# ronantakizawa/cudabulletproof

Measured on AMD Instinct MI355X. Metric: 64-bit range-proof verifies/sec (batched), higher is better.
Workload: dtype u64

## Files before the change

### cudabulletproof_amd/csrc/bp_capi.hip

```cpp
#include <hip/hip_runtime.h>
#include <map>
#include <tuple>
#include <mutex>
#include <string>
#include <vector>
#include <cstdio>
#include <cstdlib>
#include <cstring>
#include <algorithm>
#include <chrono>
#include <thread>

#include "../../include/cudabulletproof_hip.h"
#include "bp_kernels.h"
#include "ge25519_dev.h"

static_assert(sizeof(fe25519) == 32, "fe25519 layout");
static_assert(sizeof(ge25519) == 128, "ge25519 layout");
static_assert(sizeof(bp::fe) == 32 && sizeof(bp::ge) == 128, "device layout");
static_assert(sizeof(InnerProductProof) == 144, "InnerProductProof layout (SURVEY 8b)");
static_assert(sizeof(RangeProof) == 880, "RangeProof layout (SURVEY 8b)");

namespace {

// ... 290 lines not shown
    bp::SlotDev* host_dev = nullptr;
    int head = 0;

    struct Stages {
        int ft, m3, fin;
    };
    Stages stages(int L) const {
        Stages g;
        g.ft = L > 0 ? L + 1 : 1;
        g.m3 = range_mode == 2 ? (g.ft > 3 ? g.ft : 3) : -1;
        int last = g.ft;
        if (range_mode && last < 2) last = 2;
        if (g.m3 > last) last = g.m3;
        g.fin = last + 1;
        return g;
    }
    bool lane_tree = false, chains_first = false;
    bool defer_msm = false;
    int quad_force = -1;
    unsigned long long row_max = ROW_MAX_ITEMS, quad_max = QUAD_MAX_ITEMS, pair_max = PAIR_MAX_ITEMS;
    static constexpr size_t LANE_SORT_MIN = 64;
    bool lane_sort = true;
    int lane_sort_mask = 7;
    Buf sort_bins, sort_offs;
    bp::LaneSortPlan plan{};
    hipStream_t sort_s = nullptr;
    hipEvent_t ev_tick = nullptr, ev_sorted = nullptr;
    Buf ptab;
    const bp::ge* ext_tab = nullptr;
    int pbits = 0;
    const bp::ge* tables() const { return ext_tab ? ext_tab : ptab.as<bp::ge>(); }
    hipError_t init(Engine* eng, hipStream_t st, size_t mb, int nn, int range) {
        e = eng; s = st; maxB = mb; n = nn; range_mode = range;
        const char* ls = getenv("HIPBP_LANE_SORT");
        lane_sort_mask = ls ? atoi(ls) : 7;
        lane_sort = (lane_sort_mask & 7) != 0;
        const char* lt = getenv("HIPBP_LANE_TREE_MAX");
        lane_tree = n <= (lt ? atoi(lt) : bp::LANE_TREE_MAX);
        const char* cf = getenv("HIPBP_CHAINS_FIRST");
        chains_first = cf ? atoi(cf) != 0 : false;
        const char* qe = getenv("HIPBP_QUAD");
        const char* qm = getenv("HIPBP_QUAD_MAX_ITEMS");
        const char* pm = getenv("HIPBP_PAIR_MAX_ITEMS");
        quad_force = qe ? (atoi(qe) == 1 ? 4 : atoi(qe) == 2 ? 2 : atoi(qe) == 3 ? 16 : 1) : -1;
        const char* rm = getenv("HIPBP_ROW_MAX_ITEMS");
        row_max = rm ? strtoull(rm, nullptr, 10) : ROW_MAX_ITEMS;
        quad_max = qm ? strtoull(qm, nullptr, 10) : QUAD_MAX_ITEMS;
        pair_max = pm ? strtoull(pm, nullptr, 10) : PAIR_MAX_ITEMS;
        const char* dm = getenv("HIPBP_DEFER_MSM");
        defer_msm = dm && atoi(dm) != 0;
        if (const char* sp = getenv("HIPBP_DEFER_SPAN")) {
            int a = 2, b = 1, c = 0;
            if (sscanf(sp, "%d:%d:%d", &a, &b, &c) >= 1 && a >= 2) {
                defer_first = a;
                defer_last_off = b < 0 ? 0 : b;
                defer_weight = c != 0;
            }
        }
        Lr = log2i((size_t)n);
        D = stages(Lr).fin + 1;
        slots.resize(D);
        hipError_t r;
        if ((r = hipMalloc(&slots_dev, D * sizeof(bp::SlotDev))) != hipSuccess) return r;
        if ((r = hipHostMalloc(&host_dev, D * sizeof(bp::SlotDev))) != hipSuccess) return r;
        for (auto& sl : slots)
            if ((r = hipEventCreateWithFlags(&sl.copied, hipEventDisableTiming)) != hipSuccess) return r;
        const char* ss = getenv("HIPBP_SORT_STREAM");
        if (ss && atoi(ss) != 0) {
            int lo_pr = 0, hi_pr = 0;
            if ((r = hipDeviceGetStreamPriorityRange(&lo_pr, &hi_pr)) != hipSuccess) return r;
            if ((r = hipStreamCreateWithPriority(&sort_s, hipStreamNonBlocking, hi_pr)) != hipSuccess) return r;
            if ((r = hipEventCreateWithFlags(&ev_tick, hipEventDisableTiming)) != hipSuccess) return r;
            if ((r = hipEventCreateWithFlags(&ev_sorted, hipEventDisableTiming)) != hipSuccess) return r;
        }
        return hipSuccess;
    }
    void release() {
        if (s) (void)hipStreamSynchronize(s);
        for (auto& sl : slots) {
            for (auto& b : sl.b) if (b.p) (void)hipFree(b.p);
            if (sl.copied) (void)hipEventDestroy(sl.copied);
        }
        if (slots_dev) (void)hipFree(slots_dev);
        if (host_dev) (void)hipHostFree(host_dev);
        if (sort_s) (void)hipStreamSynchronize(sort_s);
        if (sort_s) (void)hipStreamDestroy(sort_s);
        if (ev_tick) (void)hipEventDestroy(ev_tick);
        if (ev_sorted) (void)hipEventDestroy(ev_sorted);
        if (sort_bins.p) (void)hipFree(sort_bins.p);
        if (sort_offs.p) (void)hipFree(sort_offs.p);
        if (ptab.p) (void)hipFree(ptab.p);
    }
    hipError_t plan_sort(Slot& sl, int idx) {
        plan = bp::LaneSortPlan{};
        bp::SlotDev& d = sl.dev;
        d.perm0 = nullptr;
        for (auto& q : d.permr) q = nullptr;
        d.perm_ft = nullptr;
        const unsigned long long B = d.bv.B;
        const int L = d.bv.L_len;
        if (!lane_sort || B < LANE_SORT_MIN) return hipSuccess;
        struct S { int kind, r; unsigned long long items; };
        S sets[bp::LANE_SORT_SETS];
        int cnt = 0;
        const bp::Stage0Lanes z = bp::stage0_lanes(B, n, L, range_mode);
        for (int c = 0; c < 4; c++)
            if (z.size[c] && (lane_sort_mask & 1)) sets[cnt++] = {bp::SS_STAGE0, c, z.size[c]};
        for (int r = 1; r < L; r++)
            if (bp::round_per_lane(n, r) && (lane_sort_mask & 2))
                sets[cnt++] = {bp::SS_ROUND, r, B * 4 * (unsigned long long)(n >> (r + 1))};
        if (lane_sort_mask & 4) sets[cnt++] = {bp::SS_FT, 0, B * 2};
        if (!cnt) return hipSuccess;
        plan.longest_first = (lane_sort_mask & 8) ? 0 : 1;
        unsigned long long total = 0;
        for (int k = 0; k < cnt; k++) total += sets[k].items;
        if (total > 0xFFFFFFFFull) return hipSuccess;
        hipError_t r;
        if ((r = sl.b[20].need(total * sizeof(uint32_t))) != hipSuccess) return r;
        const size_t nb = (size_t)bp::LANE_SORT_SETS * bp::MSM_BINS * sizeof(unsigned);
        if (!sort_bins.p) {
            if ((r = sort_bins.need(nb)) != hipSuccess) return r;
            if ((r = hipMemsetAsync(sort_bins.p, 0, nb, s)) != hipSuccess) return r;
            if ((r = sort_offs.need(nb)) != hipSuccess) return r;
        }
        uint32_t* base = sl.b[20].as<uint32_t>();
        unsigned blk = 0;
        for (int k = 0; k < cnt; k++) {
            bp::LaneSortPlan::Set& st = plan.set[k];
            st.kind = sets[k].kind; st.r = sets[k].r; st.items = sets[k].items; st.perm = base; st.block0 = blk;
            if (st.kind == bp::SS_STAGE0 && !d.perm0) d.perm0 = base;
            else if (st.kind == bp::SS_ROUND) d.permr[st.r] = base;
            else d.perm_ft = base;
            base += sets[k].items;
            blk += (unsigned)((sets[k].items + bp::LANE_SORT_BLOCK - 1) / bp::LANE_SORT_BLOCK);
        }
        plan.count = cnt;
        plan.blocks = blk;
        plan.slot = slots_dev + idx;
        return hipSuccess;
    }
    bool busy() const {
        for (auto& sl : slots) if (sl.active) return true;
        return false;
    }
    bool defer_ok() const { return range_mode != 0 && lane_tree && Lr >= 2 && 2 * Lr + 5 <= bp::MAX_REGIONS; }
    int defer_first = 2, defer_last_off = 0, defer_weight = 0;
    int msm_last(int L) const { return L - defer_last_off > defer_first ? L - defer_last_off : defer_first; }
    void msm_chunk(unsigned long long total, int L, int st, unsigned long long& lo, unsigned long long& hi) const {
        const int m = msm_last(L) - defer_first + 1, k = st - defer_first;
        auto cut = [&](int j) -> unsigned long long {
            if (j >= m) return total;
            const unsigned long long num = defer_weight ? (1ull << j) - 1 : (unsigned long long)j;
            const unsigned long long den = defer_weight ? (1ull << m) - 1 : (unsigned long long)m;
            return (total / 64 * num / den) * 64;
        };
        lo = cut(k);
        hi = cut(k + 1);
    }
    int ltree_stage(const Slot& sl, const Stages& g) const {
        return sl.dev.defer ? msm_last(sl.dev.bv.L_len) + 1 : std::min(3, g.fin - 1);
    }
// ... 28 lines not shown
    int push(const hipbp_proof_batch* b, const ge25519* P_in, uint8_t* ok, ge25519* P_out, ge25519* chk,
             uint8_t* flags_out = nullptr, ge25519* poly_out = nullptr) {
        EventTimer* tm = e->timer.on ? &e->timer : nullptr;
        bool has = b && b->count > 0;
        Slot& nw = slots[head];
        if (has) {
            int rc = check_batch(b, range_mode);
            if (rc != HIPBP_OK) return rc;
            if ((int)b->n != n) { g_err = "batch n differs from the pipeline's"; return HIPBP_ERR_ARG; }
            if (nw.active) { g_err = "pipeline slot busy (internal)"; return HIPBP_ERR_ARG; }
            BP_RET_ON(carve(nw, b->count, b->L_len));
            nw.dev.bv = view_of(b);
            nw.dev.ok = ok;
            nw.dev.P_out = (bp::ge*)P_out;
            nw.dev.chk_out = (bp::ge*)chk;
            nw.dev.flags_out = flags_out;
            nw.dev.poly_out = (bp::ge*)poly_out;
            nw.dev.range_mode = range_mode;
            nw.dev.lane_tree = lane_tree ? 1 : 0;
            nw.dev.ptab = pbits ? tables() : nullptr;
            nw.dev.pbits = pbits;
            nw.dev.defer = (defer_msm && defer_ok() && (int)b->L_len >= 2 &&
                            msm_last((int)b->L_len) + 1 < stages((int)b->L_len).fin) ? 1 : 0;
            BP_RET_ON(plan_sort(nw, head));
            BP_RET_ON(hipEventSynchronize(nw.copied));
            host_dev[head] = nw.dev;
            BP_RET_ON(hipMemcpyAsync(slots_dev + head, host_dev + head, sizeof(bp::SlotDev), hipMemcpyHostToDevice, s));
            BP_RET_ON(hipEventRecord(nw.copied, s));
            if (!range_mode)
                BP_RET_ON(hipMemcpyAsync(nw.dev.ws.Pin, P_in, b->count * sizeof(ge25519), hipMemcpyDeviceToDevice, s));
            nw.active = true;
            nw.stage = 0;
            nw.B = b->count;
        }
        bp::RegionList tr{};
        bool overflow = false;
        auto add = [&overflow](bp::RegionList& rl, int kind, int slot, int r, unsigned long long items, unsigned align) {
            if (!items) return;
            if (rl.count == bp::MAX_REGIONS) { overflow = true; return; }
            bp::Region& g = rl.reg[rl.count++];
            g.kind = kind; g.slot = slot; g.r = r; g.begin = rl.total; g.items = items;
            rl.total += (items + align - 1) & ~(unsigned long long)(align - 1);
        };
        const int chain_pass = chains_first ? 1 : 3;
        for (int pass = 0; pass < 4; pass++) {
            for (int k = 0; k < D; k++) {
                int idx = (head - k + D) % D;
// ... 18 lines not shown
                    }
                    if (st >= 2 && st <= L) add(tr, bp::RK_ROUND, idx, st - 1, B * 4 * (n >> st), 64);
                    if (sl.dev.defer && st >= defer_first && st <= msm_last(L)) {
                        unsigned long long lo, hi;
                        msm_chunk(bp::stage0_lanes(B, n, L, range_mode, bp::S0_DEFER).total, L, st, lo, hi);
                        add(tr, bp::RK_MSMT, idx, (int)lo, hi - lo, 64);
                    }
                    if (st == g.ft) add(tr, bp::RK_FINAL_TERMS, idx, 0, B * 2, 64);
                    if (st == g.m3) add(tr, bp::RK_M3, idx, 0, B * 2, 64);
                }
            }
        }
        if (overflow) { g_err = "pipeline region list overflow (internal)"; return HIPBP_ERR_ARG; }
        unsigned long long sm_items = 0;
        for (int k = 0; k < tr.count; k++)
            if (bp::region_is_sm(tr.reg[k].kind)) sm_items += tr.reg[k].items;
        int ql = sm_items <= row_max ? 16 : sm_items <= quad_max ? 4 : sm_items <= pair_max ? 2 : 1;
        if (!sm_items) {
            unsigned long long chain_items = 0;
            for (int k = 0; k < tr.count; k++) chain_items += tr.reg[k].items;
            ql = chain_items <= row_max ? 16 : 4;
        }
        if (quad_force >= 0) ql = quad_force;
        if (ql > 1) {
            unsigned long long tot = 0;
            for (int k = 0; k < tr.count; k++) {
                bp::Region& g = tr.reg[k];
                g.items *= bp::region_lanes(g.kind, ql);
                g.begin = tot;
                const unsigned long long al = g.kind == bp::RK_TREE ? 256 : 64;
                tot += (g.items + al - 1) & ~(al - 1);
            }
            tr.total = tot;
        }
        if (tr.total >= (1ull << 32)) { g_err = "pipeline tick exceeds 2^32 lanes (batch too large for n)"; return HIPBP_ERR_ARG; }
        if (tm) tm->mark(bp::KT_TERMS, false, s);
        bp::launch_terms(tr, slots_dev, G, H, g ? g : h, h, e->dtab, e->two_i, s, ql);
        if (tm) tm->mark(bp::KT_TERMS, true, s);
        BP_RET_ON(hipGetLastError());
        if (has && plan.count) {
            if (sort_s) {
                BP_RET_ON(hipEventRecord(ev_tick, s));
                BP_RET_ON(hipStreamWaitEvent(sort_s, ev_tick, 0));
                bp::launch_lane_sort(plan, sort_bins.as<unsigned>(), sort_offs.as<unsigned>(), sort_s);
                BP_RET_ON(hipGetLastError());
                BP_RET_ON(hipEventRecord(ev_sorted, sort_s));
                BP_RET_ON(hipStreamWaitEvent(s, ev_sorted, 0));
            } else {
                bp::launch_lane_sort(plan, sort_bins.as<unsigned>(), sort_offs.as<unsigned>(), s);
                BP_RET_ON(hipGetLastError());
            }
        }
        for (auto& sl : slots) {
            if (!sl.active) continue;
            if (sl.stage == stages(sl.dev.bv.L_len).fin) sl.active = false;
            else sl.stage++;
        }
        head = (head + 1) % D;
        return HIPBP_OK;
    }
    int flush() {
        while (busy()) {
            int rc = push(nullptr, nullptr, nullptr, nullptr, nullptr);
            if (rc != HIPBP_OK) return rc;
        }
        return HIPBP_OK;
    }
};

hipError_t msm_run(Engine& e, bp::ge* results, const bp::fe* scalars, const bp::ge* points, size_t n, size_t count,
                   hipStream_t s, const bp::ge* ptab = nullptr, int K = 0) {
    const size_t tot = n * count, nb = count * ((n + 255) / 256);
    Buf* w = e.msm_bufs(s);
    hipError_t err;
    if ((err = w[0].need(tot * sizeof(bp::ge))) != hipSuccess) return err;
// ... 1424 lines not shown
```

### cudabulletproof_amd/csrc/bp_kernels.h

```cpp
#pragma once
#include <hip/hip_runtime.h>
#include <stddef.h>
#include <stdint.h>

namespace bp {
struct fe;
struct ge;

struct BatchView {
    int B;
    int n;
    int ab_len;
    int L_len;
    const ge* V;
    const ge* A;
    const ge* S;
    const ge* T1;
    const ge* T2;
    const fe* t;
    const fe* a;
    const fe* b;
    const fe* c;
    const fe* x;
    const ge* L;
// ... 18 lines not shown
    ge* Pin;
    fe* psc;
    ge* pterm;
    ge* lr;
    fe* chal;
    ge* m3;
    uint8_t* rflags;
    ge* pbase;
};

struct SlotDev {
    BatchView bv;
    VerifyWs ws;
    uint8_t* ok;
    ge* P_out;
    ge* chk_out;
    uint8_t* flags_out;
    ge* poly_out;
    int range_mode;
    int lane_tree;
    uint32_t* perm0;
    uint32_t* permr[17];
    uint32_t* perm_ft;
    const ge* ptab;
    int pbits;
    int defer;
};

struct Stage0Lanes {
    unsigned long long U;
    unsigned long long off[4], size[4];
    unsigned long long total;
    unsigned long long pl;
};
enum Stage0Sel { S0_ALL = 0, S0_CRIT = 1, S0_DEFER = 2 };
__host__ __device__ inline Stage0Lanes stage0_lanes(unsigned long long B, int n, int L, int range_mode, int sel = S0_ALL) {
    Stage0Lanes z;
    const unsigned long long msm = range_mode ? B * 2 * n : 0, fold = L > 0 ? B * 2 * n : 0;
    const bool uni = n >= 64;
    const bool m = sel != S0_CRIT, f = sel != S0_DEFER;
    z.U = uni ? (m ? msm / 2 : 0) + (f ? fold : 0) : 0;
    z.size[0] = m ? (uni ? msm / 2 : msm) : 0;
    z.size[1] = f && !uni ? fold : 0;
    z.size[2] = m ? B * 2 : 0;
    z.size[3] = f && range_mode == 2 ? B * 7 : 0;
    unsigned long long o = z.U, pl = 0;
// ... 23 lines not shown
    const int n = sd.bv.n, ln = log2n(n);
    const Stage0Lanes z = stage0_lanes(B, n, sd.bv.L_len, sd.range_mode, sel);
    if (l < (uint32_t)z.U) {
        const uint32_t nG = (sd.range_mode && sel != S0_CRIT) ? B << ln : 0;
        if (l < nG) return ((l >> ln) << (ln + 1)) + (l & (n - 1));
        return (sd.range_mode ? B << (ln + 1) : 0) + (l - nG);
    }
    const Stage0Lanes za = sel == S0_ALL ? z : stage0_lanes(B, n, sd.bv.L_len, sd.range_mode);
    int c = 0;
    uint32_t base = 0;
#pragma unroll
    for (int k = 1; k < 4; k++)
        if (l >= (uint32_t)z.off[k]) { c = k; base += (uint32_t)za.size[k - 1]; }
    const uint32_t j = l - (uint32_t)z.off[c];
    if (j >= (uint32_t)z.size[c]) return UINT32_MAX;
    return stage0_class_item(sd, c, sd.perm0 ? sd.perm0[base + j] : j);
}

__host__ __device__ inline bool round_per_lane(int n, int r) { return (n >> r) < 64; }

constexpr int MSM_BINS = 513;

enum SortSetKind { SS_STAGE0 = 0, SS_ROUND = 1, SS_FT = 2 };
constexpr int LANE_SORT_SETS = 18;
constexpr int LANE_SORT_BLOCK = 256;
struct LaneSortPlan {
    int count;
    int pad;
    const SlotDev* slot;
    struct Set {
        int kind, r;
        unsigned long long items;
        uint32_t* perm;
        unsigned block0;
        unsigned pad;
    } set[LANE_SORT_SETS];
    unsigned blocks;
    int longest_first;
};
void launch_lane_sort(const LaneSortPlan& plan, unsigned* bins, unsigned* offs, hipStream_t s);

enum RegionKind { RK_STAGE0 = 0, RK_ROUND = 1, RK_FINAL_TERMS = 2, RK_FINAL = 4, RK_PREP = 5,
                  RK_TREE = 6, RK_POLY = 7, RK_M3 = 8,
                  RK_LTREE = 9 ,
                  RK_MSMT = 10  };
struct Region {
    int kind;
    int slot;
    int r;
    int pad;
    unsigned long long begin;
    unsigned long long items;
};
constexpr int LANE_TREE_MAX = 64;
constexpr int MAX_REGIONS = 24;
struct RegionList {
    int count;
    int pad;
    unsigned long long total;
    Region reg[MAX_REGIONS];
};

enum KernelKind { KT_PREP = 0, KT_TERMS, KT_TREE, KT_COMBINE, KT_COUNT };

void launch_prefix_tables(ge* tab, const ge* G, const ge* H, const ge* h, const ge* g, int n, int K, hipStream_t s);
void launch_terms(const RegionList& rl, const SlotDev* slots, const ge* G, const ge* H, const ge* g, const ge* h,
                  const ge* dtab, const fe* two_i, hipStream_t s, int ql = 1);
void launch_upload(void* dst, const void* src, size_t bytes, hipStream_t s);
#define BP_DECL_TERMS(Q)                                                                                    \
    void launch_terms##Q(const RegionList& rl, const SlotDev* slots, const ge* G, const ge* H, const ge* g,  \
                         const ge* h, const ge* dtab, const fe* two_i, hipStream_t s, unsigned lds_pad);
BP_DECL_TERMS(1)
BP_DECL_TERMS(2)
BP_DECL_TERMS(4)
BP_DECL_TERMS(16)
#undef BP_DECL_TERMS
inline bool region_is_sm(int kind) {
    return kind == RK_STAGE0 || kind == RK_ROUND || kind == RK_FINAL_TERMS || kind == RK_M3 || kind == RK_MSMT;
}
inline int region_lanes(int kind, int ql) {
    if (region_is_sm(kind)) return ql;
    return (ql >= 4 && (kind == RK_FINAL || kind == RK_LTREE || kind == RK_PREP)) ? 4 : 1;
}

constexpr size_t MSM_SORT_MIN = 4096;
void launch_msm_points(ge* pts, const fe* scal, const ge* P, size_t m, uint32_t* perm, unsigned* bins,
                       const ge* dtab, hipStream_t s, size_t pm = 0, const ge* ptab = nullptr, int K = 0);
void launch_tree(ge* out, const ge* in, int S, size_t m, hipStream_t s);
void launch_ops_scan(unsigned* bins, int longest_first, hipStream_t s);
hipError_t msm_pippenger(ge* result, const fe* scal, const ge* P, size_t n, size_t count, int c, const ge* dtab,
                         hipStream_t s);
hipError_t msm_pippenger_windows(ge* Sw, const fe* scal, const ge* P, size_t n, int c, int w0, int w1,
                                 const ge* dtab, hipStream_t s);
hipError_t pippenger_horner(ge* result, const ge* Sw, size_t count, int c, hipStream_t s);
hipError_t pippenger_release(hipStream_t s);



struct ProveIn {
    int B, n, L;
    const fe* v;
    const fe* gamma;
    const fe* sL;
    const fe* sR;
    const fe* rnd;
// ... 74 lines not shown
```

### cudabulletproof_amd/csrc/bp_kernels.hip

```cpp
#include "bp_kernels.h"
#include "ge25519_dev.h"
#include "ge25519_quad.h"
#include "sha256_dev.h"

namespace bp {

constexpr int TPB = 256;
#ifndef BP_TERMS_OCC
#define BP_TERMS_OCC 4
#endif


__device__ __forceinline__ size_t gid() { return (size_t)blockIdx.x * blockDim.x + threadIdx.x; }

__global__ __launch_bounds__(TPB) void k_prefix_tables(ge* tab, const ge* __restrict__ G, const ge* __restrict__ H,
                                                       const ge* __restrict__ h, const ge* __restrict__ g, int n,
                                                       int K, size_t total) {
    const size_t i = gid();
    if (i >= total) return;
    const size_t b = i >> K;
    const uint32_t p = (uint32_t)(i & ((1ull << K) - 1));
    const ge* P = b < (size_t)n ? &G[b] : b < 2 * (size_t)n ? &H[b - n] : b == 2 * (size_t)n ? h : g;
    if (!P) return;
    const geq q = ge_prep(*P);
// ... 105 lines not shown
}

__global__ __launch_bounds__(TPB) void k_tree(ge* out, const ge* __restrict__ in, size_t m, int nb) {
    __shared__ ge sh[TPB];
    int seg = blockIdx.x / nb, chunk = blockIdx.x % nb;
    int tid = threadIdx.x;
    size_t base = (size_t)seg * m + (size_t)chunk * TPB;
    int cnt = (int)min((size_t)TPB, m - (size_t)chunk * TPB);
    if (tid < cnt) sh[tid] = in[base + tid];
    __syncthreads();
    for (int st = 1; st < cnt; st <<= 1) {
        const int i = 2 * st * tid;
        if (i + st < cnt) sh[i] = ge_norm_dev(ge_add(sh[i], sh[i + st]));
        __syncthreads();
    }
    if (tid == 0) out[blockIdx.x] = sh[0];
}

void launch_tree(ge* out, const ge* in, int S, size_t m, hipStream_t s) {
    int nb = (int)((m + TPB - 1) / TPB);
    k_tree<<<S * nb, TPB, 0, s>>>(out, in, m, nb);
}

__device__ __forceinline__ int lane_key(const SlotDev& sd, int kind, int r, size_t j) {
    const BatchView& bv = sd.bv;
    const VerifyWs& ws = sd.ws;
    const size_t B = bv.B;
    const int n = bv.n, Lr = bv.L_len;
    fe s;
    int K = 0;
    if (kind == SS_STAGE0) {
        size_t i = stage0_class_item(sd, r, (uint32_t)j);
        if (sd.ptab) K = sd.pbits;
        const size_t nA = sd.range_mode ? B * 2 * n : 0, nB = Lr > 0 ? B * 2 * n : 0;
        if (i < nA) {
            size_t seg = i / n, p = seg >> 1;
            s = (seg & 1) ? ws.sH[p * n + i % n] : ws.sG[p];
        } else if (i - nA < nB) {
            i -= nA;
            size_t p = i / (2 * n);
            int grp = (int)(i % (2 * n)) / (n >> 1);
            s = grp < 2 ? ws.uinv[p * Lr] : ws.u[p * Lr];
        } else if (i - nA - nB < 2 * B) {
            i -= nA + nB;
            bool isC = i & 1;
            if (!isC && !sd.range_mode) return 0;
            s = ws.sc[(i >> 1) * 4 + (isC ? 3 : 0)];
        } else {
            i -= nA + nB + 2 * B;
            s = ws.psc[(i / 7) * 8 + i % 7];
            const int k = (int)(i % 7);
            if (k == 2 || k == 5 || k == 6) K = 0;
        }
    } else if (kind == SS_ROUND) {
        const int np = n >> (r + 1);
        size_t p = j / (4 * np);
        int grp = (int)(j % (4 * np)) / np;
        s = grp < 2 ? ws.uinv[p * Lr + r] : ws.u[p * Lr + r];
    } else {
        s = ws.sc[(j >> 1) * 4 + ((j & 1) ? 2 : 1)];
    }
    return sm_ops_prefix(s, K);
}

__device__ __forceinline__ int lane_set_of(const LaneSortPlan& pl, unsigned b, LaneSortPlan::Set& st) {
    int idx = 0;
    st = pl.set[0];
#pragma unroll
    for (int k = 1; k < LANE_SORT_SETS; k++)
        if (k < pl.count && b >= pl.set[k].block0) { st = pl.set[k]; idx = k; }
    return idx;
}

__global__ __launch_bounds__(LANE_SORT_BLOCK) void k_lane_hist(LaneSortPlan pl, unsigned* bins) {
    __shared__ unsigned h[OPS_BINS];
    for (int k = threadIdx.x; k < OPS_BINS; k += LANE_SORT_BLOCK) h[k] = 0;
    __syncthreads();
    LaneSortPlan::Set st;
    const int si = lane_set_of(pl, blockIdx.x, st);
    const size_t j = (size_t)(blockIdx.x - st.block0) * LANE_SORT_BLOCK + threadIdx.x;
    if (j < st.items) atomicAdd(&h[lane_key(*pl.slot, st.kind, st.r, j)], 1u);
    __syncthreads();
    for (int k = threadIdx.x; k < OPS_BINS; k += LANE_SORT_BLOCK)
        if (h[k]) atomicAdd(&bins[si * OPS_BINS + k], h[k]);
}

constexpr int LS_PER = (OPS_BINS + LANE_SORT_BLOCK - 1) / LANE_SORT_BLOCK;
__global__ __launch_bounds__(LANE_SORT_BLOCK) void k_lane_scan(unsigned* bins, unsigned* offs, int longest_first) {
    __shared__ unsigned wsum[LANE_SORT_BLOCK / 64];
    const int t = threadIdx.x;
    unsigned* bb = bins + (size_t)blockIdx.x * OPS_BINS;
    unsigned v[LS_PER], sum = 0;
#pragma unroll
    for (int u = 0; u < LS_PER; u++) {
        const int p = LS_PER * t + u, k = longest_first ? OPS_BINS - 1 - p : p;
        v[u] = p < OPS_BINS ? bb[k] : 0u;
        sum += v[u];
    }
    unsigned inc = sum;
#pragma unroll
    for (int d = 1; d < 64; d <<= 1) {
        const unsigned x = __shfl_up(inc, d, 64);
        if ((t & 63) >= d) inc += x;
    }
    if ((t & 63) == 63) wsum[t >> 6] = inc;
    __syncthreads();
    unsigned run = inc - sum;
    for (int w = 0; w < (t >> 6); w++) run += wsum[w];
#pragma unroll
    for (int u = 0; u < LS_PER; u++) {
        const int p = LS_PER * t + u, k = longest_first ? OPS_BINS - 1 - p : p;
        if (p < OPS_BINS) {
            offs[(size_t)blockIdx.x * OPS_BINS + k] = run;
            bb[k] = 0;
        }
        run += v[u];
    }
}

__global__ __launch_bounds__(LANE_SORT_BLOCK) void k_lane_scatter(LaneSortPlan pl, unsigned* offs) {
    __shared__ unsigned cnt[OPS_BINS], base[OPS_BINS];
    for (int k = threadIdx.x; k < OPS_BINS; k += LANE_SORT_BLOCK) cnt[k] = 0;
    __syncthreads();
    LaneSortPlan::Set st;
    const int si = lane_set_of(pl, blockIdx.x, st);
    const size_t j = (size_t)(blockIdx.x - st.block0) * LANE_SORT_BLOCK + threadIdx.x;
    int key = 0;
    unsigned rank = 0;
    if (j < st.items) {
        key = lane_key(*pl.slot, st.kind, st.r, j);
        rank = atomicAdd(&cnt[key], 1u);
    }
    __syncthreads();
    for (int k = threadIdx.x; k < OPS_BINS; k += LANE_SORT_BLOCK)
        if (cnt[k]) base[k] = atomicAdd(&offs[si * OPS_BINS + k], cnt[k]);
    __syncthreads();
    if (j < st.items) st.perm[base[key] + rank] = (uint32_t)j;
}

void launch_lane_sort(const LaneSortPlan& plan, unsigned* bins, unsigned* offs, hipStream_t s) {
    if (!plan.count || !plan.blocks) return;
    k_lane_hist<<<plan.blocks, LANE_SORT_BLOCK, 0, s>>>(plan, bins);
    k_lane_scan<<<plan.count, LANE_SORT_BLOCK, 0, s>>>(bins, offs, plan.longest_first);
    k_lane_scatter<<<plan.blocks, LANE_SORT_BLOCK, 0, s>>>(plan, offs);
}

static inline unsigned nblk(size_t items) { return (unsigned)((items + TPB - 1) / TPB); }

void launch_terms(const RegionList& rl, const SlotDev* slots, const ge* G, const ge* H, const ge* g, const ge* h,
                  const ge* dtab, const fe* two_i, hipStream_t s, int ql) {
    if (!rl.total) return;
    static const unsigned pad = [] { const char* e = getenv("HIPBP_TERMS_LDS_PAD"); return e ? (unsigned)atoi(e) : 0u; }();
    if (ql == 16) launch_terms16(rl, slots, G, H, g, h, dtab, two_i, s, pad);
    else if (ql == 4) launch_terms4(rl, slots, G, H, g, h, dtab, two_i, s, pad);
    else if (ql == 2) launch_terms2(rl, slots, G, H, g, h, dtab, two_i, s, pad);
    else launch_terms1(rl, slots, G, H, g, h, dtab, two_i, s, pad);
}


__global__ __launch_bounds__(TPB) void k_field_op(int op, fe* r, const fe* __restrict__ a, const fe* __restrict__ b,
                                                  size_t count) {
    size_t i = gid();
    if (op == 10 || op == 12) {
        i >>= 2;
        if (i >= count) return;
        const fe z = op == 10 ? fe_mul_q4(a[i], b[i]) : fe_mul_q4_k(a[i]);
        if ((threadIdx.x & 3) == 0) r[i] = z;
        return;
    }
// ... 219 lines not shown
```

### cudabulletproof_amd/csrc/bp_verify_dev.h

```cpp
#pragma once
#include "bp_kernels.h"
#include "ge25519_dev.h"
#include "ge25519_quad.h"
#include "sha256_dev.h"

namespace bp {

#ifndef BP_TERMS_OCC
#define BP_TERMS_OCC 4
#endif
constexpr int TPB = 256;
__device__ __forceinline__ size_t gid() { return (size_t)blockIdx.x * blockDim.x + threadIdx.x; }



__device__ __forceinline__ void prep_std_task(const BatchView& bv, const VerifyWs& ws, const fe* __restrict__ two_i,
                                              size_t p, const fe& z, const fe& z2, const fe& sy) {
    const int n = bv.n;
    fe x = chal_x(bv.T1[p], bv.T2[p]);
    const fe two = fe_add(fe_set(1), fe_set(1));
    fe z3 = fe_mul(z2, z);
    fe t1 = fe_mul(fe_sub(z, z2), sy);
    fe s2 = fe_set(1);
    for (int i = 1; i < n; i++) s2 = fe_add(s2, two_i[i]);
// ... 114 lines not shown
            tr = u;
        }
        const bool me = (r & 3) == qd;
        const int k = r >> 2;
        m0 = fe_sel(me && k == 0, u, m0);
        m1 = fe_sel(me && k == 1, u, m1);
        m2 = fe_sel(me && k == 2, u, m2);
        m3 = fe_sel(me && k == 3, u, m3);
    }
#pragma unroll
    for (int k = 0; k < 4; k++) {
        const int r = 4 * k + qd;
        const fe u = k == 0 ? m0 : k == 1 ? m1 : k == 2 ? m2 : m3;
        if (r < Lr) {
            ws.u[p * Lr + r] = fe_canon(u);
            ws.uinv[p * Lr + r] = fe_canon(fe_invert(u));
        }
    }
    if (qd == 0) {
        ws.ipok[p] = fe_eq(fe_canon(acc), fe_canon(bv.c[p])) ? 1 : 0;
        ws.sc[p * 4 + 1] = fe_canon(bv.a[p * abl]);
        ws.sc[p * 4 + 2] = fe_canon(bv.b[p * abl]);
        ws.sc[p * 4 + 3] = fe_canon(bv.c[p]);
    }
}

__device__ __forceinline__ ge folded_point(const VerifyWs& ws, int n, int r, size_t p, bool isH, int m) {
    const int npp = n >> r;
    const ge* f = ws.fold[(r - 1) & 1] + p * (2 * n);
    if (!isH) return ge_norm_host(ge_add(f[m], f[2 * npp + m]));
    return ge_norm_host(ge_add(f[3 * npp + m], f[npp + m]));
}

struct SmJob {
    fe s;
    ge P;
    ge* dst;
    int dev_norm;
    int base;
};


__device__ __forceinline__ void fold_job(const BatchView& bv, const VerifyWs& ws, int r, uint32_t p, uint32_t k,
                                         const ge* __restrict__ G, const ge* __restrict__ H, SmJob& jb) {
    const int n = bv.n, lnp = log2n(n) - r - 1, np = 1 << lnp, Lr = bv.L_len;
    const int grp = (int)(k >> lnp), j = (int)(k & (np - 1));
// ... 250 lines not shown
    if (i >= rl.total) return;
    const Region rg = find_region(rl, i);
    size_t l = i - rg.begin;
    const SlotDev& sd = slots[rg.slot];
    if (rg.kind == RK_TREE) {
        ge* sh = reinterpret_cast<ge*>(qs);
        const int n = sd.bv.n, ch = n < TPB ? n : TPB, tid = threadIdx.x, idx = tid & (ch - 1);
        const bool live = l < rg.items;
        if (live) sh[tid] = sd.ws.msm_pts[l];
        __syncthreads();
        for (int st = 1; st < ch; st <<= 1) {
            const int j = tid - idx + 2 * st * idx;
            if (live && 2 * st * idx + st < ch) sh[j] = ge_norm_dev(ge_add(sh[j], sh[j + st]));
            __syncthreads();
        }
        if (live && idx == 0) {
            if (n <= TPB) sd.ws.msm_part[l / n] = sh[tid];
            else sd.ws.msm_pts[l] = sh[tid];
        }
        return;
    }
    if (l >= rg.items) return;
    if (rg.kind == RK_PREP) {
        const size_t B = sd.bv.B;
        if (QL >= 4) {
            const size_t it = l >> 2;
            const int qd = threadIdx.x & 3;
            if (sd.range_mode && it < B) prep_range_task_q4(sd.bv, sd.ws, two_i, it, sd.range_mode, qd);
            else prep_ipa_task_q4(sd.bv, sd.ws, sd.range_mode ? it - B : it, qd);
        } else if (sd.range_mode && l < B) {
            prep_range_task(sd.bv, sd.ws, two_i, l, sd.range_mode);
        } else {
            prep_ipa_task(sd.bv, sd.ws, sd.range_mode ? l - B : l);
        }
    } else if (rg.kind == RK_POLY) {
        poly_task(sd, l);
    } else if (rg.kind == RK_FINAL) {
        if (QL >= 4) final_task<true>(sd, l >> 2);
        else final_task<false>(sd, l);
    } else if (rg.kind == RK_LTREE) {
        if (QL >= 4) ltree_task<true>(sd, l >> 2);
        else ltree_task<false>(sd, l);
    } else {
        SmJob jb;
        jb.base = -1;
        bool live = true;
        uint32_t li = (uint32_t)l;
        if (QL == 16) li >>= 4;
        if (QL == 4) li >>= 2;
        if (QL == 2) li >>= 1;
        if (rg.kind == RK_STAGE0 || rg.kind == RK_MSMT) {
            const uint32_t it = rg.kind == RK_MSMT ? stage0_item(sd, (uint32_t)rg.r + li, S0_DEFER)
                                                   : stage0_item(sd, li, sd.defer ? S0_CRIT : S0_ALL);
            live = it != UINT32_MAX && stage0_job(sd, it, G, H, g, h, jb);
        } else if (rg.kind == RK_M3) {
            m3_job(sd, li, jb);
// ... 37 lines not shown
```

Before: 210,200.

## Fuse lane-sort permutation building into prep kernel with per-block local sort

Drops the separate histogram, scan and scatter lane-sort kernels and their global bin buffers and optional side stream. Each prep block now sorts the MSM lanes of its own group of proofs in LDS, right after the prep work, and writes the permutation directly. Prep lanes are re-laid out as whole 256-thread groups split into range and IPA parts, so every thread reaches the block barriers. This saves three launches and the global atomics per step. In exchange the ordering becomes block-local rather than batch-wide, and the serial per-set sort loop lengthens the prep kernel.

New measurement: 210,600 (median of 6 runs). No clear change (+0.2%).

```diff
diff --git a/cudabulletproof_amd/csrc/bp_capi.hip b/cudabulletproof_amd/csrc/bp_capi.hip
--- a/cudabulletproof_amd/csrc/bp_capi.hip
+++ b/cudabulletproof_amd/csrc/bp_capi.hip
@@ -336,10 +336,6 @@
     static constexpr size_t LANE_SORT_MIN = 64;
     bool lane_sort = true;
     int lane_sort_mask = 7;
-    Buf sort_bins, sort_offs;
-    bp::LaneSortPlan plan{};
-    hipStream_t sort_s = nullptr;
-    hipEvent_t ev_tick = nullptr, ev_sorted = nullptr;
     Buf ptab;
     const bp::ge* ext_tab = nullptr;
     int pbits = 0;
@@ -379,14 +375,6 @@
         if ((r = hipHostMalloc(&host_dev, D * sizeof(bp::SlotDev))) != hipSuccess) return r;
         for (auto& sl : slots)
             if ((r = hipEventCreateWithFlags(&sl.copied, hipEventDisableTiming)) != hipSuccess) return r;
-        const char* ss = getenv("HIPBP_SORT_STREAM");
-        if (ss && atoi(ss) != 0) {
-            int lo_pr = 0, hi_pr = 0;
-            if ((r = hipDeviceGetStreamPriorityRange(&lo_pr, &hi_pr)) != hipSuccess) return r;
-            if ((r = hipStreamCreateWithPriority(&sort_s, hipStreamNonBlocking, hi_pr)) != hipSuccess) return r;
-            if ((r = hipEventCreateWithFlags(&ev_tick, hipEventDisableTiming)) != hipSuccess) return r;
-            if ((r = hipEventCreateWithFlags(&ev_sorted, hipEventDisableTiming)) != hipSuccess) return r;
-        }
         return hipSuccess;
     }
     void release() {
@@ -397,60 +385,34 @@
         }
         if (slots_dev) (void)hipFree(slots_dev);
         if (host_dev) (void)hipHostFree(host_dev);
-        if (sort_s) (void)hipStreamSynchronize(sort_s);
-        if (sort_s) (void)hipStreamDestroy(sort_s);
-        if (ev_tick) (void)hipEventDestroy(ev_tick);
-        if (ev_sorted) (void)hipEventDestroy(ev_sorted);
-        if (sort_bins.p) (void)hipFree(sort_bins.p);
-        if (sort_offs.p) (void)hipFree(sort_offs.p);
         if (ptab.p) (void)hipFree(ptab.p);
     }
-    hipError_t plan_sort(Slot& sl, int idx) {
-        plan = bp::LaneSortPlan{};
+    hipError_t plan_sort(Slot& sl) {
         bp::SlotDev& d = sl.dev;
         d.perm0 = nullptr;
         for (auto& q : d.permr) q = nullptr;
         d.perm_ft = nullptr;
+        d.lane_sort = 0;
         const unsigned long long B = d.bv.B;
         const int L = d.bv.L_len;
         if (!lane_sort || B < LANE_SORT_MIN) return hipSuccess;
-        struct S { int kind, r; unsigned long long items; };
-        S sets[bp::LANE_SORT_SETS];
-        int cnt = 0;
-        const bp::Stage0Lanes z = bp::stage0_lanes(B, n, L, range_mode);
-        for (int c = 0; c < 4; c++)
-            if (z.size[c] && (lane_sort_mask & 1)) sets[cnt++] = {bp::SS_STAGE0, c, z.size[c]};
+        const unsigned long long pl = (lane_sort_mask & 1) ? bp::stage0_lanes(B, n, L, range_mode).pl : 0;
+        unsigned long long total = pl + ((lane_sort_mask & 4) ? B * 2 : 0);
         for (int r = 1; r < L; r++)
             if (bp::round_per_lane(n, r) && (lane_sort_mask & 2))
-                sets[cnt++] = {bp::SS_ROUND, r, B * 4 * (unsigned long long)(n >> (r + 1))};
-        if (lane_sort_mask & 4) sets[cnt++] = {bp::SS_FT, 0, B * 2};
-        if (!cnt) return hipSuccess;
-        plan.longest_first = (lane_sort_mask & 8) ? 0 : 1;
-        unsigned long long total = 0;
-        for (int k = 0; k < cnt; k++) total += sets[k].items;
+                total += B * bp::lane_set_per_proof(bp::SS_ROUND, r, n, L, range_mode);
         if (total > 0xFFFFFFFFull) return hipSuccess;
         hipError_t r;
         if ((r = sl.b[20].need(total * sizeof(uint32_t))) != hipSuccess) return r;
-        const size_t nb = (size_t)bp::LANE_SORT_SETS * bp::MSM_BINS * sizeof(unsigned);
-        if (!sort_bins.p) {
-            if ((r = sort_bins.need(nb)) != hipSuccess) return r;
-            if ((r = hipMemsetAsync(sort_bins.p, 0, nb, s)) != hipSuccess) return r;
-            if ((r = sort_offs.need(nb)) != hipSuccess) return r;
-        }
         uint32_t* base = sl.b[20].as<uint32_t>();
-        unsigned blk = 0;
-        for (int k = 0; k < cnt; k++) {
-            bp::LaneSortPlan::Set& st = plan.set[k];
-            st.kind = sets[k].kind; st.r = sets[k].r; st.items = sets[k].items; st.perm = base; st.block0 = blk;
-            if (st.kind == bp::SS_STAGE0 && !d.perm0) d.perm0 = base;
-            else if (st.kind == bp::SS_ROUND) d.permr[st.r] = base;
-            else d.perm_ft = base;
-            base += sets[k].items;
-            blk += (unsigned)((sets[k].items + bp::LANE_SORT_BLOCK - 1) / bp::LANE_SORT_BLOCK);
-        }
-        plan.count = cnt;
-        plan.blocks = blk;
-        plan.slot = slots_dev + idx;
+        if (pl) { d.perm0 = base; base += pl; }
+        for (int k = 1; k < L; k++)
+            if (bp::round_per_lane(n, k) && (lane_sort_mask & 2)) {
+                d.permr[k] = base;
+                base += B * bp::lane_set_per_proof(bp::SS_ROUND, k, n, L, range_mode);
+            }
+        if (lane_sort_mask & 4) d.perm_ft = base;
+        d.lane_sort = (lane_sort_mask & 8) ? 2 : 1;
         return hipSuccess;
     }
     bool busy() const {
@@ -525,7 +487,7 @@
             nw.dev.pbits = pbits;
             nw.dev.defer = (defer_msm && defer_ok() && (int)b->L_len >= 2 &&
                             msm_last((int)b->L_len) + 1 < stages((int)b->L_len).fin) ? 1 : 0;
-            BP_RET_ON(plan_sort(nw, head));
+            BP_RET_ON(plan_sort(nw));
             BP_RET_ON(hipEventSynchronize(nw.copied));
             host_dev[head] = nw.dev;
             BP_RET_ON(hipMemcpyAsync(slots_dev + head, host_dev + head, sizeof(bp::SlotDev), hipMemcpyHostToDevice, s));
@@ -590,13 +552,19 @@
             ql = chain_items <= row_max ? 16 : 4;
         }
         if (quad_force >= 0) ql = quad_force;
-        if (ql > 1) {
+        {
             unsigned long long tot = 0;
             for (int k = 0; k < tr.count; k++) {
                 bp::Region& g = tr.reg[k];
-                g.items *= bp::region_lanes(g.kind, ql);
+                const bool prep = g.kind == bp::RK_PREP;
+                const unsigned long long al = (g.kind == bp::RK_TREE || prep) ? 256 : 64;
+                if (prep) {
+                    tot = (tot + al - 1) & ~(al - 1);
+                    g.items = bp::prep_lanes(slots[g.slot].dev.bv.B, range_mode, ql);
+                } else {
+                    g.items *= bp::region_lanes(g.kind, ql);
+                }
                 g.begin = tot;
-                const unsigned long long al = g.kind == bp::RK_TREE ? 256 : 64;
                 tot += (g.items + al - 1) & ~(al - 1);
             }
             tr.total = tot;
@@ -606,19 +574,6 @@
         bp::launch_terms(tr, slots_dev, G, H, g ? g : h, h, e->dtab, e->two_i, s, ql);
         if (tm) tm->mark(bp::KT_TERMS, true, s);
         BP_RET_ON(hipGetLastError());
-        if (has && plan.count) {
-            if (sort_s) {
-                BP_RET_ON(hipEventRecord(ev_tick, s));
-                BP_RET_ON(hipStreamWaitEvent(sort_s, ev_tick, 0));
-                bp::launch_lane_sort(plan, sort_bins.as<unsigned>(), sort_offs.as<unsigned>(), sort_s);
-                BP_RET_ON(hipGetLastError());
-                BP_RET_ON(hipEventRecord(ev_sorted, sort_s));
-                BP_RET_ON(hipStreamWaitEvent(s, ev_sorted, 0));
-            } else {
-                bp::launch_lane_sort(plan, sort_bins.as<unsigned>(), sort_offs.as<unsigned>(), s);
-                BP_RET_ON(hipGetLastError());
-            }
-        }
         for (auto& sl : slots) {
             if (!sl.active) continue;
             if (sl.stage == stages(sl.dev.bv.L_len).fin) sl.active = false;
diff --git a/cudabulletproof_amd/csrc/bp_kernels.h b/cudabulletproof_amd/csrc/bp_kernels.h
--- a/cudabulletproof_amd/csrc/bp_kernels.h
+++ b/cudabulletproof_amd/csrc/bp_kernels.h
@@ -64,6 +64,7 @@
     uint32_t* perm0;
     uint32_t* permr[17];
     uint32_t* perm_ft;
+    int lane_sort;
     const ge* ptab;
     int pbits;
     int defer;
@@ -133,23 +134,53 @@
 constexpr int MSM_BINS = 513;
 
 enum SortSetKind { SS_STAGE0 = 0, SS_ROUND = 1, SS_FT = 2 };
-constexpr int LANE_SORT_SETS = 18;
-constexpr int LANE_SORT_BLOCK = 256;
-struct LaneSortPlan {
-    int count;
-    int pad;
-    const SlotDev* slot;
-    struct Set {
-        int kind, r;
-        unsigned long long items;
-        uint32_t* perm;
-        unsigned block0;
-        unsigned pad;
-    } set[LANE_SORT_SETS];
-    unsigned blocks;
-    int longest_first;
-};
-void launch_lane_sort(const LaneSortPlan& plan, unsigned* bins, unsigned* offs, hipStream_t s);
+
+constexpr int PREP_BLOCK = 256;
+__host__ __device__ inline uint32_t prep_group_proofs(int ql) { return ql >= 4 ? PREP_BLOCK / 4 : PREP_BLOCK; }
+__host__ __device__ inline unsigned long long prep_groups(unsigned long long B, int ql) {
+    const unsigned long long gp = prep_group_proofs(ql);
+    return (B + gp - 1) / gp;
+}
+__host__ __device__ inline unsigned long long prep_lanes(unsigned long long B, int range_mode, int ql) {
+    return (range_mode ? 2 : 1) * prep_groups(B, ql) * PREP_BLOCK;
+}
+struct PrepLane {
+    int part;
+    uint32_t group;
+    uint32_t p;
+    int qd;
+};
+__host__ __device__ inline PrepLane prep_lane(uint32_t B, int range_mode, int ql, uint32_t l) {
+    const uint32_t ng = (uint32_t)prep_groups(B, ql), blk = l / PREP_BLOCK, t = l % PREP_BLOCK;
+    PrepLane z;
+    z.part = range_mode ? (blk >= ng ? 1 : 0) : 1;
+    z.group = range_mode && blk >= ng ? blk - ng : blk;
+    z.p = z.group * prep_group_proofs(ql) + (ql >= 4 ? t >> 2 : t);
+    z.qd = ql >= 4 ? (int)(t & 3) : 0;
+    return z;
+}
+__host__ __device__ inline void prep_group_range(uint32_t B, int ql, uint32_t g, uint32_t& p0, uint32_t& p1) {
+    const uint32_t gp = prep_group_proofs(ql);
+    p0 = g * gp < B ? g * gp : B;
+    p1 = p0 + gp < B ? p0 + gp : B;
+}
+__host__ __device__ inline uint32_t lane_set_per_proof(int kind, int r, int n, int L, int range_mode) {
+    if (kind == SS_STAGE0) {
+        if (r == 0) return range_mode ? (n >= 64 ? n : 2 * n) : 0;
+        if (r == 1) return (L > 0 && n < 64) ? 2 * n : 0;
+        if (r == 2) return 2;
+        return range_mode == 2 ? 7 : 0;
+    }
+    if (kind == SS_ROUND) return 4u * (uint32_t)(n >> (r + 1));
+    return 2;
+}
+__host__ __device__ inline int lane_set_part(int kind, int r) { return kind == SS_STAGE0 && (r == 0 || r == 3) ? 0 : 1; }
+__host__ __device__ inline int lane_sort_bin(int key, int shortest_first) { return shortest_first ? key : MSM_BINS - 1 - key; }
+__host__ __device__ inline uint32_t perm0_base(uint32_t B, int n, int L, int range_mode, int c) {
+    uint32_t base = 0;
+    for (int k = 0; k < c; k++) base += B * lane_set_per_proof(SS_STAGE0, k, n, L, range_mode);
+    return base;
+}
 
 enum RegionKind { RK_STAGE0 = 0, RK_ROUND = 1, RK_FINAL_TERMS = 2, RK_FINAL = 4, RK_PREP = 5,
                   RK_TREE = 6, RK_POLY = 7, RK_M3 = 8,
@@ -191,7 +222,7 @@
 }
 inline int region_lanes(int kind, int ql) {
     if (region_is_sm(kind)) return ql;
-    return (ql >= 4 && (kind == RK_FINAL || kind == RK_LTREE || kind == RK_PREP)) ? 4 : 1;
+    return (ql >= 4 && (kind == RK_FINAL || kind == RK_LTREE)) ? 4 : 1;
 }
 
 constexpr size_t MSM_SORT_MIN = 4096;
diff --git a/cudabulletproof_amd/csrc/bp_kernels.hip b/cudabulletproof_amd/csrc/bp_kernels.hip
--- a/cudabulletproof_amd/csrc/bp_kernels.hip
+++ b/cudabulletproof_amd/csrc/bp_kernels.hip
@@ -151,129 +151,6 @@
     k_tree<<<S * nb, TPB, 0, s>>>(out, in, m, nb);
 }
 
-__device__ __forceinline__ int lane_key(const SlotDev& sd, int kind, int r, size_t j) {
-    const BatchView& bv = sd.bv;
-    const VerifyWs& ws = sd.ws;
-    const size_t B = bv.B;
-    const int n = bv.n, Lr = bv.L_len;
-    fe s;
-    int K = 0;
-    if (kind == SS_STAGE0) {
-        size_t i = stage0_class_item(sd, r, (uint32_t)j);
-        if (sd.ptab) K = sd.pbits;
-        const size_t nA = sd.range_mode ? B * 2 * n : 0, nB = Lr > 0 ? B * 2 * n : 0;
-        if (i < nA) {
-            size_t seg = i / n, p = seg >> 1;
-            s = (seg & 1) ? ws.sH[p * n + i % n] : ws.sG[p];
-        } else if (i - nA < nB) {
-            i -= nA;
-            size_t p = i / (2 * n);
-            int grp = (int)(i % (2 * n)) / (n >> 1);
-            s = grp < 2 ? ws.uinv[p * Lr] : ws.u[p * Lr];
-        } else if (i - nA - nB < 2 * B) {
-            i -= nA + nB;
-            bool isC = i & 1;
-            if (!isC && !sd.range_mode) return 0;
-            s = ws.sc[(i >> 1) * 4 + (isC ? 3 : 0)];
-        } else {
-            i -= nA + nB + 2 * B;
-            s = ws.psc[(i / 7) * 8 + i % 7];
-            const int k = (int)(i % 7);
-            if (k == 2 || k == 5 || k == 6) K = 0;
-        }
-    } else if (kind == SS_ROUND) {
-        const int np = n >> (r + 1);
-        size_t p = j / (4 * np);
-        int grp = (int)(j % (4 * np)) / np;
-        s = grp < 2 ? ws.uinv[p * Lr + r] : ws.u[p * Lr + r];
-    } else {
-        s = ws.sc[(j >> 1) * 4 + ((j & 1) ? 2 : 1)];
-    }
-    return sm_ops_prefix(s, K);
-}
-
-__device__ __forceinline__ int lane_set_of(const LaneSortPlan& pl, unsigned b, LaneSortPlan::Set& st) {
-    int idx = 0;
-    st = pl.set[0];
-#pragma unroll
-    for (int k = 1; k < LANE_SORT_SETS; k++)
-        if (k < pl.count && b >= pl.set[k].block0) { st = pl.set[k]; idx = k; }
-    return idx;
-}
-
-__global__ __launch_bounds__(LANE_SORT_BLOCK) void k_lane_hist(LaneSortPlan pl, unsigned* bins) {
-    __shared__ unsigned h[OPS_BINS];
-    for (int k = threadIdx.x; k < OPS_BINS; k += LANE_SORT_BLOCK) h[k] = 0;
-    __syncthreads();
-    LaneSortPlan::Set st;
-    const int si = lane_set_of(pl, blockIdx.x, st);
-    const size_t j = (size_t)(blockIdx.x - st.block0) * LANE_SORT_BLOCK + threadIdx.x;
-    if (j < st.items) atomicAdd(&h[lane_key(*pl.slot, st.kind, st.r, j)], 1u);
-    __syncthreads();
-    for (int k = threadIdx.x; k < OPS_BINS; k += LANE_SORT_BLOCK)
-        if (h[k]) atomicAdd(&bins[si * OPS_BINS + k], h[k]);
-}
-
-constexpr int LS_PER = (OPS_BINS + LANE_SORT_BLOCK - 1) / LANE_SORT_BLOCK;
-__global__ __launch_bounds__(LANE_SORT_BLOCK) void k_lane_scan(unsigned* bins, unsigned* offs, int longest_first) {
-    __shared__ unsigned wsum[LANE_SORT_BLOCK / 64];
-    const int t = threadIdx.x;
-    unsigned* bb = bins + (size_t)blockIdx.x * OPS_BINS;
-    unsigned v[LS_PER], sum = 0;
-#pragma unroll
-    for (int u = 0; u < LS_PER; u++) {
-        const int p = LS_PER * t + u, k = longest_first ? OPS_BINS - 1 - p : p;
-        v[u] = p < OPS_BINS ? bb[k] : 0u;
-        sum += v[u];
-    }
-    unsigned inc = sum;
-#pragma unroll
-    for (int d = 1; d < 64; d <<= 1) {
-        const unsigned x = __shfl_up(inc, d, 64);
-        if ((t & 63) >= d) inc += x;
-    }
-    if ((t & 63) == 63) wsum[t >> 6] = inc;
-    __syncthreads();
-    unsigned run = inc - sum;
-    for (int w = 0; w < (t >> 6); w++) run += wsum[w];
-#pragma unroll
-    for (int u = 0; u < LS_PER; u++) {
-        const int p = LS_PER * t + u, k = longest_first ? OPS_BINS - 1 - p : p;
-        if (p < OPS_BINS) {
-            offs[(size_t)blockIdx.x * OPS_BINS + k] = run;
-            bb[k] = 0;
-        }
-        run += v[u];
-    }
-}
-
-__global__ __launch_bounds__(LANE_SORT_BLOCK) void k_lane_scatter(LaneSortPlan pl, unsigned* offs) {
-    __shared__ unsigned cnt[OPS_BINS], base[OPS_BINS];
-    for (int k = threadIdx.x; k < OPS_BINS; k += LANE_SORT_BLOCK) cnt[k] = 0;
-    __syncthreads();
-    LaneSortPlan::Set st;
-    const int si = lane_set_of(pl, blockIdx.x, st);
-    const size_t j = (size_t)(blockIdx.x - st.block0) * LANE_SORT_BLOCK + threadIdx.x;
-    int key = 0;
-    unsigned rank = 0;
-    if (j < st.items) {
-        key = lane_key(*pl.slot, st.kind, st.r, j);
-        rank = atomicAdd(&cnt[key], 1u);
-    }
-    __syncthreads();
-    for (int k = threadIdx.x; k < OPS_BINS; k += LANE_SORT_BLOCK)
-        if (cnt[k]) base[k] = atomicAdd(&offs[si * OPS_BINS + k], cnt[k]);
-    __syncthreads();
-    if (j < st.items) st.perm[base[key] + rank] = (uint32_t)j;
-}
-
-void launch_lane_sort(const LaneSortPlan& plan, unsigned* bins, unsigned* offs, hipStream_t s) {
-    if (!plan.count || !plan.blocks) return;
-    k_lane_hist<<<plan.blocks, LANE_SORT_BLOCK, 0, s>>>(plan, bins);
-    k_lane_scan<<<plan.count, LANE_SORT_BLOCK, 0, s>>>(bins, offs, plan.longest_first);
-    k_lane_scatter<<<plan.blocks, LANE_SORT_BLOCK, 0, s>>>(plan, offs);
-}
-
 static inline unsigned nblk(size_t items) { return (unsigned)((items + TPB - 1) / TPB); }
 
 void launch_terms(const RegionList& rl, const SlotDev* slots, const ge* G, const ge* H, const ge* g, const ge* h,
diff --git a/cudabulletproof_amd/csrc/bp_verify_dev.h b/cudabulletproof_amd/csrc/bp_verify_dev.h
--- a/cudabulletproof_amd/csrc/bp_verify_dev.h
+++ b/cudabulletproof_amd/csrc/bp_verify_dev.h
@@ -160,6 +160,106 @@
         ws.sc[p * 4 + 1] = fe_canon(bv.a[p * abl]);
         ws.sc[p * 4 + 2] = fe_canon(bv.b[p * abl]);
         ws.sc[p * 4 + 3] = fe_canon(bv.c[p]);
+    }
+}
+
+__device__ __forceinline__ int lane_key(const SlotDev& sd, int kind, int r, uint32_t j) {
+    const BatchView& bv = sd.bv;
+    const VerifyWs& ws = sd.ws;
+    const int n = bv.n, ln = log2n(n), Lr = bv.L_len;
+    fe s;
+    int K = sd.ptab ? sd.pbits : 0;
+    if (kind == SS_STAGE0) {
+        if (r == 0) {
+            if (n >= 64) {
+                s = ws.sH[j];
+            } else {
+                const uint32_t seg = j >> ln;
+                s = (seg & 1) ? ws.sH[(size_t)(seg >> 1) * n + (j & (n - 1))] : ws.sG[seg >> 1];
+            }
+        } else if (r == 1) {
+            const uint32_t p = j >> (ln + 1);
+            const int grp = (int)(j & (2 * n - 1)) / (n >> 1);
+            s = grp < 2 ? ws.uinv[(size_t)p * Lr] : ws.u[(size_t)p * Lr];
+        } else if (r == 2) {
+            const bool isC = j & 1;
+            if (!isC && !sd.range_mode) return 0;
+            s = isC ? ws.sc[(size_t)(j >> 1) * 4 + 3] : fe_canon(bv.t[j >> 1]);
+        } else {
+            const uint32_t p = j / 7u;
+            const int k = (int)(j - 7u * p);
+            s = ws.psc[(size_t)p * 8 + k];
+            if (k == 2 || k == 5 || k == 6) K = 0;
+        }
+    } else if (kind == SS_ROUND) {
+        const int l4 = ln - r + 1;
+        const uint32_t p = j >> l4;
+        const int grp = (int)(j & ((1u << l4) - 1)) >> (l4 - 2);
+        s = grp < 2 ? ws.uinv[(size_t)p * Lr + r] : ws.u[(size_t)p * Lr + r];
+        K = 0;
+    } else {
+        s = ws.sc[(size_t)(j >> 1) * 4 + ((j & 1) ? 2 : 1)];
+        K = 0;
+    }
+    return sm_ops_prefix(s, K);
+}
+
+constexpr int LS_PER = (MSM_BINS + PREP_BLOCK - 1) / PREP_BLOCK;
+__device__ __forceinline__ void lane_sort_group(const SlotDev& sd, int kind, int r, uint32_t* __restrict__ perm,
+                                                uint32_t lo, uint32_t hi, unsigned* lds) {
+    const int t = threadIdx.x, sf = sd.lane_sort == 2;
+    unsigned* bins = lds;
+    unsigned* wsum = lds + MSM_BINS;
+    for (int k = t; k < MSM_BINS; k += PREP_BLOCK) bins[k] = 0;
+    __syncthreads();
+    for (uint32_t j = lo + t; j < hi; j += PREP_BLOCK) atomicAdd(&bins[lane_sort_bin(lane_key(sd, kind, r, j), sf)], 1u);
+    __syncthreads();
+    unsigned v[LS_PER], sum = 0;
+#pragma unroll
+    for (int u = 0; u < LS_PER; u++) {
+        const int b = LS_PER * t + u;
+        v[u] = b < MSM_BINS ? bins[b] : 0u;
+        sum += v[u];
+    }
+    unsigned inc = sum;
+#pragma unroll
+    for (int d = 1; d < 64; d <<= 1) {
+        const unsigned x = __shfl_up(inc, d, 64);
+        if ((t & 63) >= d) inc += x;
+    }
+    if ((t & 63) == 63) wsum[t >> 6] = inc;
+    __syncthreads();
+    unsigned run = lo + inc - sum;
+    for (int w = 0; w < (t >> 6); w++) run += wsum[w];
+#pragma unroll
+    for (int u = 0; u < LS_PER; u++) {
+        const int b = LS_PER * t + u;
+        if (b < MSM_BINS) bins[b] = run;
+        run += v[u];
+    }
+    __syncthreads();
+    for (uint32_t j = lo + t; j < hi; j += PREP_BLOCK)
+        perm[atomicAdd(&bins[lane_sort_bin(lane_key(sd, kind, r, j), sf)], 1u)] = j;
+    __syncthreads();
+}
+
+__device__ __forceinline__ void lane_sort_block(const SlotDev& sd, int part, uint32_t p0, uint32_t p1, unsigned* lds) {
+    const uint32_t B = (uint32_t)sd.bv.B;
+    const int n = sd.bv.n, L = sd.bv.L_len, mode = sd.range_mode;
+    __syncthreads();
+    if (sd.perm0) {
+        for (int c = 0; c < 4; c++) {
+            const uint32_t per = lane_set_per_proof(SS_STAGE0, c, n, L, mode);
+            if (per && lane_set_part(SS_STAGE0, c) == part)
+                lane_sort_group(sd, SS_STAGE0, c, sd.perm0 + perm0_base(B, n, L, mode, c), p0 * per, p1 * per, lds);
+        }
+    }
+    if (part == 1) {
+        for (int r = 1; r < L; r++) {
+            const uint32_t per = lane_set_per_proof(SS_ROUND, r, n, L, mode);
+            if (sd.permr[r]) lane_sort_group(sd, SS_ROUND, r, sd.permr[r], p0 * per, p1 * per, lds);
+        }
+        if (sd.perm_ft) lane_sort_group(sd, SS_FT, 0, sd.perm_ft, p0 * 2, p1 * 2, lds);
     }
 }
 
@@ -456,16 +556,22 @@
     }
     if (l >= rg.items) return;
     if (rg.kind == RK_PREP) {
-        const size_t B = sd.bv.B;
-        if (QL >= 4) {
-            const size_t it = l >> 2;
-            const int qd = threadIdx.x & 3;
-            if (sd.range_mode && it < B) prep_range_task_q4(sd.bv, sd.ws, two_i, it, sd.range_mode, qd);
-            else prep_ipa_task_q4(sd.bv, sd.ws, sd.range_mode ? it - B : it, qd);
-        } else if (sd.range_mode && l < B) {
-            prep_range_task(sd.bv, sd.ws, two_i, l, sd.range_mode);
-        } else {
-            prep_ipa_task(sd.bv, sd.ws, sd.range_mode ? l - B : l);
+        const uint32_t B = (uint32_t)sd.bv.B;
+        const PrepLane pl = prep_lane(B, sd.range_mode, QL, (uint32_t)l);
+        if (pl.p < B) {
+            if (QL >= 4) {
+                if (pl.part == 0) prep_range_task_q4(sd.bv, sd.ws, two_i, pl.p, sd.range_mode, pl.qd);
+                else prep_ipa_task_q4(sd.bv, sd.ws, pl.p, pl.qd);
+            } else if (pl.part == 0) {
+                prep_range_task(sd.bv, sd.ws, two_i, pl.p, sd.range_mode);
+            } else {
+                prep_ipa_task(sd.bv, sd.ws, pl.p);
+            }
+        }
+        if (sd.lane_sort) {
+            uint32_t p0, p1;
+            prep_group_range(B, QL, pl.group, p0, p1);
+            lane_sort_block(sd, pl.part, p0, p1, reinterpret_cast<unsigned*>(qs));
         }
     } else if (rg.kind == RK_POLY) {
         poly_task(sd, l);
```
